# pyannote/pyannote-audio

Hardware: AMD Instinct MI355X
Metric: audio-hours/sec (real-time factor) for speaker-diarization-3.1 pipeline (higher is better)
Workload: dtype f32

## Files before the change

include/pyannote_amd.h:

```cpp
#ifndef PYANNOTE_AMD_H
#define PYANNOTE_AMD_H

#include <stddef.h>
#include <stdint.h>

#ifdef __cplusplus
extern "C" {
#endif

int pa_version(void);
const char* pa_last_error(void);

void pa_prof_enable(int on);
size_t pa_prof_report(char* buf, size_t cap);

#define PA_MAX_LSTM_LAYERS 8
#define PA_MAX_LINEAR 4

typedef struct pa_seg_weights {
  int32_t sinc_stride;
  int32_t lstm_layers;
  int32_t lstm_hidden;
  int32_t lstm_bidir;
  int32_t num_linear;
// ... 101 lines not shown
                   int num_chunks, int num_samples, const float* masks, int num_masks, int mask_frames,
                   const int32_t* nearest_idx, float* emb, void* workspace, size_t workspace_bytes,
                   void* stream);

size_t pa_emb_ragged_workspace_bytes(const pa_emb_weights* w, int num_utterances, int max_samples);
int pa_emb_forward_ragged(const pa_emb_weights* w, const float* wav, int64_t wav_len, const int64_t* offsets,
                          const int32_t* lengths, int num_utterances, int max_samples, const float* masks, float* emb,
                          void* workspace, size_t workspace_bytes, void* stream);

size_t pa_emb_calibrate_workspace_bytes(const pa_emb_weights* w, int num_chunks, int num_samples);
int pa_emb_calibrate_winograd(const pa_emb_weights* w, const float* wav, int64_t wav_len, int64_t chunk_stride,
                              int num_chunks, int num_samples, float* report, float* emb, void* workspace,
                              size_t workspace_bytes, void* stream);
int pa_absmax_diff(const float* got, const float* ref, long n, float* out2, void* stream);

int pa_fbank(const float* wav, long wav_len, long chunk_stride, int B, int N, const float* window,
             const float* tw256, const float* tw512, const float* mel_w, const int* mel_lo,
             const int* mel_hi, int nmel, float* out, int center, void* stream);
int pa_fbank_center_span(const float* fb, int B, int T, int nmel, int kernel, float* out, void* stream);
int pa_resnet_stem(const float* fbank, int B, int T, int F, const float* w9, const float* shift,
                   float* out, void* stream);
int pa_conv3x3(const float* X, int B, int H, int W, int cin, const float* Wg, const float* shift,
               const float* R, float* Y, int cout, int stride, int relu, void* stream);
int pa_winograd_pack_host(const float* conv_weight ,
                          const float* bn_scale , int cout, int cin,
                          float* U_slabs );
int pa_conv3x3_wino(const float* X, int B, int H, int W, int cin, const float* U, const float* shift,
                    const float* R, float* Y, int cout, int relu, void* stream);
int pa_winograd4_pack_host(const float* conv_weight ,
                           const float* bn_scale , int cout, int cin,
                           float* U_slabs );
int pa_conv3x3_wino4(const float* X, int B, int H, int W, int cin, const float* U, const float* shift,
                     const float* R, float* Y, int cout, int relu, void* stream);
int pa_conv3x3_wino4_rows(const float* X, int B, int H, int W, int cin, const float* U, const float* shift,
                          const float* R, float* Y, int cout, int relu, int rows, void* stream);
int pa_conv3x3_wino_rows(const float* X, int B, int H, int W, int cin, const float* U, const float* shift,
                         const float* R, float* Y, int cout, int relu, int y_first, void* stream);
int pa_stats_pool(const float* feat, int B, int Fh, int Tp, int C, const float* masks, int S, int Fm,
                  const int* nearest_idx, float* stats, void* stream);
int pa_fbank_ragged(const float* wav, long wav_len, const int64_t* offsets, const int32_t* lengths, int B,
                    int max_samples, const float* window, const float* tw256, const float* tw512, const float* mel_w,
                    const int* mel_lo, const int* mel_hi, int nmel, float* out, void* stream);
int pa_zero_tail_cols(float* x, int B, int H, int W, int C, const int32_t* lengths, int halvings, void* stream);
int pa_stats_pool_ragged(const float* feat, int B, int Fh, int W, int C, const int32_t* lengths, int halvings,
                         const float* masks, int ld_masks, float* stats, void* stream);

// ... 281 lines not shown
```

pyannote-audio_amd/csrc/emb_conv_s2.hip:

```cpp
#include "common.h"
#include "emb_conv_s2_geom.h"

namespace pa {

typedef __attribute__((address_space(3))) unsigned char* cs2_lds_t;
typedef const volatile f32x4 __attribute__((address_space(3))) * cs2_lds_f32x4_ptr;
__device__ __forceinline__ f32x4 cs2_lds_read128(cs2_lds_t p) { return *(cs2_lds_f32x4_ptr)p; }

__device__ __forceinline__ void cs2_barrier() {
  asm volatile("s_waitcnt lgkmcnt(0)" ::: "memory");
  __builtin_amdgcn_s_barrier();
  asm volatile("" ::: "memory");
}

#define CS2_STR2(x) #x
#define CS2_STR(x) CS2_STR2(x)
#define CS2_TAIL_WAIT_LIT 32
static_assert(ConvS2Geom<4, 1>::TILE_STORES == CS2_TAIL_WAIT_LIT && ConvS2Geom<2, 2>::TILE_STORES == CS2_TAIL_WAIT_LIT,
              "the literal of the s_waitcnt string");
static_assert(ConvS2Geom<4, 1>::NPW <= CS2_SLOTS && ConvS2Geom<2, 2>::NPW <= CS2_SLOTS, "a slot of the MFMA run per piece");

template <int IMM>
__device__ __forceinline__ void cs2_piece(unsigned dst, int voff, __amdgpu_buffer_rsrc_t srd, int soff) {
  asm volatile("s_add_u32 m0, %0, %1\n\ts_nop 0\n\tbuffer_load_dwordx4 %2, %3, %4 offen lds"
               :: "s"(dst), "i"(IMM), "v"(voff), "s"(srd), "s"(soff)
               : "memory", "scc");
}
__device__ __forceinline__ void cs2_piece_s(unsigned dst, int delta, int voff, __amdgpu_buffer_rsrc_t srd, int soff) {
  asm volatile("s_add_u32 m0, %0, %1\n\ts_nop 0\n\tbuffer_load_dwordx4 %2, %3, %4 offen lds"
               :: "s"(dst), "s"(delta), "v"(voff), "s"(srd), "s"(soff)
               : "memory", "scc");
}
struct Cs2Stage {
  __amdgpu_buffer_rsrc_t xsrd, wsrd;
  int soff;
  unsigned pdst, wdst;
  int last_delta;
};
template <class G, int N>
__device__ __forceinline__ void cs2_issue(const Cs2Stage& st, const int (&poff)[G::PPW], const int (&woff)[G::WPW]) {
  if constexpr (N < G::PPW - 1) cs2_piece<4096 * N>(st.pdst, poff[N], st.xsrd, st.soff);
  else if constexpr (N == G::PPW - 1) cs2_piece_s(st.pdst, st.last_delta, poff[N], st.xsrd, st.soff);
  else if constexpr (N < G::NPW) cs2_piece<4096 * (N - G::PPW)>(st.wdst, woff[N - G::PPW], st.wsrd, st.soff);
}
template <class G>
__device__ __forceinline__ void cs2_issue_n(const int n, const Cs2Stage& st, const int (&poff)[G::PPW],
                                            const int (&woff)[G::WPW]) {
  switch (n) {
#define CS2_CASE(I) case I: cs2_issue<G, I>(st, poff, woff); break;
    CS2_CASE(0) CS2_CASE(1) CS2_CASE(2) CS2_CASE(3) CS2_CASE(4) CS2_CASE(5) CS2_CASE(6) CS2_CASE(7) CS2_CASE(8)
    CS2_CASE(9) CS2_CASE(10) CS2_CASE(11) CS2_CASE(12) CS2_CASE(13) CS2_CASE(14) CS2_CASE(15) CS2_CASE(16)
    CS2_CASE(17) CS2_CASE(18) CS2_CASE(19) CS2_CASE(20) CS2_CASE(21) CS2_CASE(22) CS2_CASE(23) CS2_CASE(24)
    CS2_CASE(25) CS2_CASE(26)
#undef CS2_CASE
    default: break;
  }
}

template <int TH, int TWT, bool HAS_R>
__global__ __launch_bounds__(256, 2) void k_conv3x3_s2(const float* __restrict__ X, int H, int W, int CIN,
                                                       const float* __restrict__ Wg,
                                                       const float* __restrict__ shift,
                                                       const float* __restrict__ R, float* __restrict__ Y, int Ho,
                                                       int Wo, int COUT, int relu, int tiles_w, int tiles_hw,
                                                       int n_tiles, int total_tiles, int xranges,
                                                       int* __restrict__ counters) {
  using G = ConvS2Geom<TH, TWT>;
  constexpr int BN = CS2_BN;
  constexpr int OOB = CS2_OOB;
  extern __shared__ __attribute__((aligned(16))) unsigned char smem_s2[];
  const cs2_lds_t lds = (cs2_lds_t)smem_s2;
  const unsigned lds0 = (unsigned)(size_t)lds;
  int* mail = reinterpret_cast<int*>(smem_s2 + G::LDS_BYTES);

  const int tid = threadIdx.x, lane = tid & 63;
  const int slw = __builtin_amdgcn_readfirstlane(tid >> 6);
  const int li = lane & 31, kh = lane >> 5;

  struct Tile {
    int b, n0, y0, x0;
  };
  const int num_pb = total_tiles / n_tiles;
  auto pair_of = [&](int t) {
    return xranges ? (t & 7) * ((num_pb + 7) >> 3) + (t >> 3) / n_tiles : ((t >> 3) / n_tiles) * 8 + (t & 7);
  };
  auto decode = [&](int t) {
    Tile q;
    const int pb = pair_of(t);
    q.n0 = (((t >> 3) % n_tiles)) * BN;
    const int pix = pb % tiles_hw;
// ... 9 lines not shown
      r = tq_claim_own(tqq);
    }
  };

  cs2_lds_t aptr[9][2];
#pragma unroll
  for (int tap = 0; tap < 9; ++tap)
#pragma unroll
    for (int h = 0; h < 2; ++h) {
      aptr[tap][h] = lds + conv_s2_a_addr<G>(slw, li, kh, h, tap);
      asm volatile("" : "+v"(aptr[tap][h]));
    }
  cs2_lds_t bptr[2];
#pragma unroll
  for (int h = 0; h < 2; ++h) {
    bptr[h] = lds + G::W_BASE + conv_s2_b_addr(0, li, kh, h, 0);
    asm volatile("" : "+v"(bptr[h]));
  }
  ConvS2Lane pl[G::PPW];
#pragma unroll
  for (int k = 0; k < G::PPW; ++k) pl[k] = conv_s2_patch_lane<G>(conv_s2_patch_piece<G>(slw, k), lane, W, CIN);
  int woff[G::WPW];
#pragma unroll
  for (int k = 0; k < G::WPW; ++k) woff[k] = conv_s2_w_lane(4 * k + slw, lane, COUT, CIN);
  const int last_delta = 1024 * (conv_s2_patch_piece<G>(slw, G::PPW - 1) - slw);
  int poff[G::PPW];
  auto tile_offsets = [&](const Tile& q) {
    const int sy = 2 * q.y0 - 1, sx = 2 * q.x0 - 1, sbase = conv_s2_tile_base(q.y0, q.x0, W, CIN);
#pragma unroll
    for (int k = 0; k < G::PPW; ++k) poff[k] = conv_s2_patch_off(pl[k], sy, sx, sbase, H, W);
  };
  auto x_srd = [&](const Tile& q, bool live) {
    return __builtin_amdgcn_make_buffer_rsrc(const_cast<float*>(X + (long)q.b * H * W * CIN), 0,
                                             live ? H * W * CIN * 4 : 0, 0x00020000);
  };
  auto w_srd = [&](const Tile& q, bool live) {
    return __builtin_amdgcn_make_buffer_rsrc(const_cast<float*>(Wg + (long)q.n0 * CIN), 0,
                                             live ? (9 * COUT - q.n0) * CIN * 4 : 0, 0x00020000);
  };
  auto stage_to = [&](int to_buf, __amdgpu_buffer_rsrc_t xs, __amdgpu_buffer_rsrc_t ws, int c0) {
    Cs2Stage st;
    st.xsrd = xs;
    st.wsrd = ws;
    st.soff = c0 * 4;
    st.pdst = lds0 + to_buf * G::PATCH_BYTES + 1024 * slw;
    st.wdst = lds0 + G::W_BASE + to_buf * G::W_BYTES + 1024 * slw;
    st.last_delta = __builtin_amdgcn_readfirstlane(last_delta);
    return st;
  };

  const TileQueue tq{counters, (int)(blockIdx.x & 7), ((num_pb + 7) >> 3) * n_tiles};
  if (tid == 0) mail[0] = resolve(tq, tq_claim_own(tq));
  __syncthreads();
  const int t0 = __builtin_amdgcn_readfirstlane(mail[0]);
  if (t0 < 0) {
    if (tid == 0) tq_done(tq, gridDim.x);
    return;
  }
  Tile cur = decode(t0), nxt = cur;
  __amdgpu_buffer_rsrc_t xcur = x_srd(cur, true), wcur = w_srd(cur, true);
  tile_offsets(cur);
  {
    const Cs2Stage st = stage_to(0, xcur, wcur, 0);
#pragma unroll
    for (int n = 0; n < G::NPW; ++n) cs2_issue_n<G>(n, st, poff, woff);
  }
  int claim = 0;
  if (tid == 0) claim = tq_claim_own(tq);
  const int nst = CIN / CS2_CB;
  int buf = 0, tpar = 1, tn = -1;
  bool first_tile = true;

  for (;;) {
    f32x16 acc[2];
#pragma unroll
    for (int j = 0; j < 2; ++j)
#pragma unroll
      for (int r = 0; r < 16; ++r) acc[j][r] = 0.f;
    for (int s = 0; s < nst; ++s) {
      const bool last = s == nst - 1;
      if (s == 0 && !first_tile) asm volatile("s_waitcnt vmcnt(" CS2_STR(CS2_TAIL_WAIT_LIT) ")" ::: "memory");
      else asm volatile("s_waitcnt vmcnt(0)" ::: "memory");
      if (last && tid == 0) mail[tpar] = resolve(tq, claim);
      cs2_barrier();
      Cs2Stage st;
      auto setup = [&]() {
        __amdgpu_buffer_rsrc_t xs = xcur, ws = wcur;
        if (last) {
          tn = __builtin_amdgcn_readfirstlane(mail[tpar]);
          if (tn >= 0) {
            nxt = decode(tn);
            tile_offsets(nxt);
          }
          xs = x_srd(nxt, tn >= 0);
          ws = w_srd(nxt, tn >= 0);
        }
        st = stage_to(buf ^ 1, xs, ws, last ? 0 : (s + 1) * CS2_CB);
      };

      {
        f32x4 fa[2][2], fb[2][2][2];
        auto rd = [&](const int tap, const int r, const int par) {
          const int h = r / 3, w = r % 3;
          if (w == 0) fa[par][h] = cs2_lds_read128(aptr[tap][h]);
          else fb[par][w - 1][h] = cs2_lds_read128(bptr[h] + tap * 4096 + (w - 1) * 2048);
        };
#pragma unroll
        for (int r = 0; r < 6; ++r) rd(0, r, 0);
        __builtin_amdgcn_sched_barrier(0);
        setup();
        __builtin_amdgcn_sched_barrier(0);
#pragma unroll
        for (int tap = 0; tap < 9; ++tap) {
          const int par = tap & 1;
#pragma unroll
          for (int m = 0; m < 16; ++m) {
            const int h = m >> 3, c = (m >> 1) & 3, j = m & 1;
            const float av = fa[par][h][c], bv = fb[par][j][h][c];
            acc[j] = MFMA32(av, bv, acc[j]);
            __builtin_amdgcn_sched_barrier(0);
            if (tap + 1 < 9 && (m & 1) == 0 && m < 12) {
              rd(tap + 1, m >> 1, par ^ 1);
              __builtin_amdgcn_sched_barrier(0);
            }
            const int slot = conv_s2_slot_of(tap, m);
            if (slot >= 0 && slot < G::NPW) {
              cs2_issue_n<G>(slot, st, poff, woff);
              __builtin_amdgcn_sched_barrier(0);
            }
          }
        }
      }
      {
        const int dp = buf ? -G::PATCH_BYTES : G::PATCH_BYTES, dw = buf ? -G::W_BYTES : G::W_BYTES;
#pragma unroll
        for (int tap = 0; tap < 9; ++tap)
#pragma unroll
          for (int h = 0; h < 2; ++h) {
            aptr[tap][h] += dp;
            asm volatile("" : "+v"(aptr[tap][h]));
          }
#pragma unroll
        for (int h = 0; h < 2; ++h) {
          bptr[h] += dw;
// ... 11 lines not shown
          const_cast<float*>(HAS_R ? R + (long)cur.b * Ho * Wo * COUT : Y), 0, Ho * Wo * COUT * 4, 0x00020000);
      const int y = cur.y0 + slw / TWT, xbase = cur.x0 + 32 * (slw % TWT) + 4 * kh;
      int off[2][16];
      float rv[2][16];
      auto goffs = [&](int j, int* o) {
        const int n = cur.n0 + 32 * j + li;
#pragma unroll
        for (int r = 0; r < 16; ++r) {
          const int x = xbase + (r & 3) + 8 * (r >> 2);
          o[r] = (y < Ho && x < Wo) ? ((y * Wo + x) * COUT + n) * 4 : OOB;
        }
      };
      auto gres = [&](const int* o, float* v) {
        if (HAS_R) {
#pragma unroll
          for (int r = 0; r < 16; ++r)
            v[r] = __builtin_bit_cast(float, __builtin_amdgcn_raw_buffer_load_b32(rsrd, o[r], 0, 0));
        } else {
#pragma unroll
          for (int r = 0; r < 16; ++r) v[r] = 0.f;
        }
      };
      const float shv[2] = {shift[cur.n0 + li], shift[cur.n0 + 32 + li]};
      goffs(0, off[0]);
      gres(off[0], rv[0]);
#pragma unroll
      for (int j = 0; j < 2; ++j) {
        if (j + 1 < 2) {
          goffs(j + 1, off[(j + 1) & 1]);
          gres(off[(j + 1) & 1], rv[(j + 1) & 1]);
        }
        const float sh = shv[j];
#pragma unroll
        for (int r = 0; r < 16; ++r) {
          float v = acc[j][r] + sh + rv[j & 1][r];
          if (relu) v = fmaxf(v, 0.f);
          __builtin_amdgcn_raw_buffer_store_b32(__builtin_bit_cast(unsigned int, v), ysrd, off[j & 1][r], 0, 0);
        }
      }
    }
    if (tn < 0) break;
    cur = nxt;
    xcur = x_srd(cur, true);
    wcur = w_srd(cur, true);
    tpar ^= 1;
  }
  if (tid == 0) tq_done(tq, gridDim.x);
}

int xcd_ranges_wanted(bool by_default);

template <int TH, int TWT, bool HAS_R>
static int launch_conv_s2_r(const float* X, int B, int H, int W, int CIN, const float* Wg, const float* shift,
                            const float* R, float* Y, int COUT, int relu, hipStream_t st) {
  using G = ConvS2Geom<TH, TWT>;
  const int Ho = (H - 1) / 2 + 1, Wo = (W - 1) / 2 + 1;
  const int tiles_w = cdiv(Wo, G::TW), tiles_h = cdiv(Ho, TH);
  const size_t lds = (size_t)G::LDS_BYTES + 16;
  constexpr int MAXDEV = 16;
  static int resident_of[MAXDEV] = {0};
  int dev = 0;
  (void)hipGetDevice(&dev);
  if (dev < 0 || dev >= MAXDEV) dev = 0;
  if (!resident_of[dev]) {
    (void)hipFuncSetAttribute((const void*)k_conv3x3_s2<TH, TWT, HAS_R>, hipFuncAttributeMaxDynamicSharedMemorySize,
                              (int)lds);
    int cus = 256;
    (void)hipDeviceGetAttribute(&cus, hipDeviceAttributeMultiprocessorCount, dev);
    resident_of[dev] = cus;
  }
  const int resident = resident_of[dev] & ~7;
  const int tiles_hw = tiles_w * tiles_h, n_tiles = COUT / CS2_BN;
  const long total = (long)tiles_hw * n_tiles * B;
  const int grid = (int)(total < resident ? total : resident);
  int* counters = tile_counters();
  if (counters == nullptr) {
    set_error("pa_conv3x3: cannot allocate the tile counters");
    return 2;
  }
  hipLaunchKernelGGL((k_conv3x3_s2<TH, TWT, HAS_R>), dim3(grid), dim3(256), lds, st, X, H, W, CIN, Wg, shift, R, Y, Ho,
                     Wo, COUT, relu, tiles_w, tiles_hw, n_tiles, (int)total, xcd_ranges_wanted(true), counters);
  return 0;
}

int launch_conv_s2(const float* X, int B, int H, int W, int CIN, const float* Wg, const float* shift, const float* R,
                   float* Y, int COUT, int relu, hipStream_t st) {
  const int Ho = (H - 1) / 2 + 1;
  if (Ho >= 16)
    return R != nullptr ? launch_conv_s2_r<4, 1, true>(X, B, H, W, CIN, Wg, shift, R, Y, COUT, relu, st)
                        : launch_conv_s2_r<4, 1, false>(X, B, H, W, CIN, Wg, shift, R, Y, COUT, relu, st);
  return R != nullptr ? launch_conv_s2_r<2, 2, true>(X, B, H, W, CIN, Wg, shift, R, Y, COUT, relu, st)
                      : launch_conv_s2_r<2, 2, false>(X, B, H, W, CIN, Wg, shift, R, Y, COUT, relu, st);
}

}
```

pyannote-audio_amd/csrc/emb_conv_s2_geom.h:

```cpp
#pragma once

namespace pa {

constexpr int CS2_CB = 16;
constexpr int CS2_BN = 64;
constexpr int CS2_OOB = (int)0x80000000;

template <int TH_, int TWT_>
struct ConvS2Geom {
  static constexpr int TH = TH_, TWT = TWT_, TW = 32 * TWT_;
  static constexpr int PH = 2 * TH + 1, PW = 2 * TW + 1;
  static constexpr int PWH = TW + 1;
  static constexpr int PENT = PH * 2 * PWH;
  static constexpr int PPIECES = (PENT + 15) / 16;
  static constexpr int WPIECES = 9 * CS2_BN / 16;
  static constexpr int PPW = (PPIECES + 3) / 4;
  static constexpr int WPW = WPIECES / 4;
  static constexpr int NPW = PPW + WPW;
  static constexpr int PATCH_BYTES = PPIECES * 1024;
  static constexpr int W_BYTES = WPIECES * 1024;
  static constexpr int W_BASE = 2 * PATCH_BYTES;
  static constexpr int LDS_BYTES = 2 * (PATCH_BYTES + W_BYTES);
  static constexpr int TILE_STORES = 2 * 16;
  static_assert(TH * TWT == 4, "one M-tile per wave, four waves");
  static_assert(WPIECES % 4 == 0 && PPW * 4 >= PPIECES, "pieces split over four waves");
  static_assert(8 * 4096 + 2048 < 65536, "ds_read immediates of a B fragment: tap and N-tile");
  static_assert(LDS_BYTES + 64 <= 160 * 1024, "two stages in LDS");
};

__device__ __forceinline__ int conv_s2_swz(int e) { return (e >> 2) & 3; }

template <class G>
__device__ __forceinline__ int conv_s2_patch_piece(int w, int k) {
  const int i = 4 * k + w;
  return i < G::PPIECES ? i : G::PPIECES - 1;
}

struct ConvS2Lane {
  int rel, py, px;
};
constexpr int CS2_NO_COLUMN = 0x20000000;
template <class G>
__device__ __forceinline__ ConvS2Lane conv_s2_patch_lane(int piece, int lane, int W, int CIN) {
  const int sl = 64 * piece + lane;
  const int e = sl >> 2, q = (sl & 3) ^ conv_s2_swz(e);
  const int plane = e / G::PWH, col = e % G::PWH;
  const int py = plane >> 1, px = 2 * col + (plane & 1);
  const bool real = e < G::PENT && px < G::PW;
  ConvS2Lane L;
  L.rel = ((py * W + px) * CIN + 4 * q) * 4;
  L.py = py;
  L.px = real ? px : CS2_NO_COLUMN;
  return L;
}
__device__ __forceinline__ int conv_s2_tile_base(int y0, int x0, int W, int CIN) {
  return ((2 * y0 - 1) * W + 2 * x0 - 1) * CIN * 4;
}
__device__ __forceinline__ int conv_s2_patch_off(const ConvS2Lane& L, int sy, int sx, int sbase, int H, int W) {
  const bool ok = (unsigned)(L.py + sy) < (unsigned)H && (unsigned)(L.px + sx) < (unsigned)W;
  return ok ? sbase + L.rel : CS2_OOB;
}
__device__ __forceinline__ int conv_s2_w_lane(int piece, int lane, int COUT, int CIN) {
  const int sl = 64 * piece + lane;
  const int e = sl >> 2, q = (sl & 3) ^ conv_s2_swz(e);
  const int tap = e >> 6, n = e & 63;
  return ((tap * COUT + n) * CIN + 4 * q) * 4;
}

template <class G>
__device__ __forceinline__ int conv_s2_a_entry(int mt, int li, int tap) {
  const int dy = tap / 3, dx = tap % 3;
  const int yy = mt / G::TWT, xt = mt % G::TWT;
  return ((2 * yy + dy) * 2 + (dx & 1)) * G::PWH + 32 * xt + li + (dx >> 1);
}
__device__ __forceinline__ int conv_s2_slot_addr(int e, int q) { return e * 64 + ((q ^ conv_s2_swz(e)) << 4); }
template <class G>
__device__ __forceinline__ int conv_s2_a_addr(int mt, int li, int kh, int h, int tap) {
  return conv_s2_slot_addr(conv_s2_a_entry<G>(mt, li, tap), 2 * kh + h);
}
__device__ __forceinline__ int conv_s2_b_addr(int j, int li, int kh, int h, int tap) {
  return conv_s2_slot_addr(tap * 64 + 32 * j + li, 2 * kh + h);
}

constexpr int CS2_SLOTS = 9 * 3;
__device__ __forceinline__ int conv_s2_slot_of(int tap, int m) {
  return (m == 3 || m == 9 || m == 15) ? tap * 3 + (m - 3) / 6 : -1;
}

}
```

pyannote-audio_amd/csrc/emb_forward.cpp:

```cpp
#include "forward_common.h"

namespace {

struct EmbPlan {
  int B, N, T, F, S;
  int Hs[5], Ws[5];
  size_t fbank, act[4], stats, total, act_elems;
  size_t t2_off, gather_off;
};

inline bool prefer_wino4(int H, int W, int cin) {
  auto up = [](int a, int b) { return (long)((a + b - 1) / b) * b; };
  long p4 = up(H, 4) * up(W, 64);
  const long p4_lin = up(H, 4) * up(W, 4);
  if (p4_lin * 120 <= p4 * 100) p4 = p4_lin * 120 / 100;
  long p2 = up(H, 8) * up(W, 32);
  if (up(H, 4) * up(W, 64) < p2) p2 = up(H, 4) * up(W, 64);
  if (up(H, 2) * up(W, 128) < p2) p2 = up(H, 2) * up(W, 128);
  const long gain = cin >= 256 ? 130 : 122;
  return p4 * 100 <= p2 * gain;
}

bool make_plan(const pa_emb_weights* w, int B, int N, int S, EmbPlan* p, bool calib = false) {
  if (N < 400) return false;
  p->B = B;
  p->N = N;
  p->S = S < 1 ? 1 : S;
  p->T = 1 + (N - 400) / 160;
  p->F = w->num_mel;
  p->Hs[0] = p->F;
  p->Ws[0] = p->T;
  for (int l = 0; l < w->num_layers; ++l) {
// ... 161 lines not shown
          pa::set_error("pa_emb_forward: block %d needs a shortcut conv but none was given", blk);
          return 3;
        }
        PA_RUN(pa_gemm_tn_ex(t2, planes, w->blk_w3[blk], planes, w->blk_shift3[blk], res, nxt, cout, B * Ho * Wo,
                             cout, planes, 2, 0, stream));
        float* t = cur;
        cur = nxt;
        nxt = t;
        cin = cout;
      }
    }
  } else
  for (int l = 0; l < w->num_layers; ++l) {
    const int cout = w->planes[l];
    for (int i = 0; i < w->num_blocks[l]; ++i, ++blk) {
      if (blk >= PA_MAX_RES_BLOCKS) {
        pa::set_error("pa_emb_forward: more than %d residual blocks", PA_MAX_RES_BLOCKS);
        return 3;
      }
      const int stride = (i == 0 && l > 0) ? 2 : 1;
      const int H = stride == 2 ? p.Hs[l] : p.Hs[l + 1], W = stride == 2 ? p.Ws[l] : p.Ws[l + 1];
      const int Ho = p.Hs[l + 1], Wo = p.Ws[l + 1];
      if (w->blk_wsc[blk] != nullptr) {
        PA_RUN(pa_conv3x3(cur, B, H, W, cin, w->blk_w1[blk], w->blk_shift1[blk], nullptr, f1, cout, stride,
                          1, stream));
        PA_RUN(zero_tail(f1, l + 1, cout));
        const size_t q = (size_t)B * Ho * Wo * cin;
        float* R = f2 + pa::Bump::align(q);
        if (stride == 2)
          PA_RUN(pa_gemm_tn_s2(cur, B, H, W, cin, w->blk_wsc[blk], cin, w->blk_shiftsc[blk], R, cout, cout, stream));
        else
          PA_RUN(pa_gemm_tn(cur, cin, w->blk_wsc[blk], cin, w->blk_shiftsc[blk], R, cout, B * Ho * Wo, cout, cin, 0, 0,
                            stream));
        PA_RUN(conv_s1(f1, Ho, Wo, cout, w->blk_v2[blk], w->blk_u2[blk], w->blk_w2[blk], w->blk_shift2[blk], R, cur,
                       cout, 2 * blk + 1));
        PA_RUN(zero_tail(cur, l + 1, cout));
      } else {
        if (stride != 1 || cin != cout) {
          pa::set_error("pa_emb_forward: block %d needs a shortcut conv but none was given", blk);
          return 3;
        }
        PA_RUN(conv_s1(cur, H, W, cin, w->blk_v1[blk], w->blk_u1[blk], w->blk_w1[blk], w->blk_shift1[blk], nullptr, f1,
                       cout, 2 * blk));
        PA_RUN(zero_tail(f1, l + 1, cout));
        PA_RUN(conv_s1(f1, H, W, cout, w->blk_v2[blk], w->blk_u2[blk], w->blk_w2[blk], w->blk_shift2[blk], cur, f2,
                       cout, 2 * blk + 1));
        PA_RUN(zero_tail(f2, l + 1, cout));
        float* t = cur;
        cur = f2;
        f2 = t;
      }
      cin = cout;
// ... 62 lines not shown
```

pyannote-audio_amd/csrc/emb_resnet.hip:

```cpp
#include "common.h"

namespace pa {

constexpr int STEM_TS = 64;
constexpr int STEM_LD = STEM_TS + 3;

__global__ __launch_bounds__(256) void k_stem(const float* __restrict__ fb, int T, int F,
                                              const float* __restrict__ w9,
                                              const float* __restrict__ shift,
                                              float* __restrict__ out) {
  extern __shared__ float xs[];
  const int b = blockIdx.y, t0 = blockIdx.x * STEM_TS;
  const int tid = threadIdx.x;
  for (int i = tid; i < 2 * STEM_LD; i += 256) xs[(i < STEM_LD ? 0 : (F + 1) * STEM_LD - STEM_LD) + i] = 0.f;
  const int n = (STEM_TS + 2) * F;
  for (int i0 = 0; i0 < n; i0 += 8 * 256) {
    float v[8];
#pragma unroll
    for (int k = 0; k < 8; ++k) {
      const int i = i0 + tid + 256 * k;
      const int tt = i / F, ff = i - tt * F, t = t0 + tt - 1;
      v[k] = (i < n && t >= 0 && t < T) ? fb[((long)b * T + t) * F + ff] : 0.f;
    }
#pragma unroll
// ... 284 lines not shown
        if (g + 1 < NG) {
          goffs(g + 1, off[(g + 1) & 1]);
          gres(off[(g + 1) & 1], rv[(g + 1) & 1]);
        }
        const int i = g / NT, j = g % NT;
        const float sh = shift[cur.n0 + 32 * j + li];
#pragma unroll
        for (int r = 0; r < 16; ++r) {
          float v = acc[i][j][r] + sh + rv[g & 1][r];
          if (relu) v = fmaxf(v, 0.f);
          __builtin_amdgcn_raw_buffer_store_b32(__builtin_bit_cast(unsigned int, v), ysrd, off[g & 1][r], 0, 0);
        }
      }
    }
    if (tn < 0) break;
    cur = nxt;
  }
  if (tid == 0) tq_done(tq, gridDim.x);
}

int xcd_ranges_wanted(bool by_default);
int launch_conv_s2(const float* X, int B, int H, int W, int CIN, const float* Wg, const float* shift, const float* R,
                   float* Y, int COUT, int relu, hipStream_t st);

template <int TH, int TWT, int BN, bool HAS_R>
static int launch_conv_r(const float* X, int B, int H, int W, int CIN, const float* Wg,
                         const float* shift, const float* R, float* Y, int COUT, int relu,
                         hipStream_t st) {
  using G = ConvGeom<TH, TWT>;
  const int Ho = H, Wo = W;
  const int tiles_w = cdiv(Wo, G::TW), tiles_h = cdiv(Ho, TH);
  const size_t lds = (size_t)(G::PATCH + 9 * BN * CLD) * sizeof(float);
  constexpr int MAXDEV = 16;
  static int resident_of[MAXDEV] = {0}, per_cu_of[MAXDEV] = {0};
  int dev = 0;
  (void)hipGetDevice(&dev);
  if (dev < 0 || dev >= MAXDEV) dev = 0;
  if (!resident_of[dev]) {
    (void)hipFuncSetAttribute((const void*)k_conv3x3<TH, TWT, BN, HAS_R>,
                              hipFuncAttributeMaxDynamicSharedMemorySize, (int)lds);
    int cus = 256, per_cu = 2;
    (void)hipDeviceGetAttribute(&cus, hipDeviceAttributeMultiprocessorCount, dev);
    if (hipOccupancyMaxActiveBlocksPerMultiprocessor(&per_cu, k_conv3x3<TH, TWT, BN, HAS_R>, 256, lds) !=
            hipSuccess || per_cu < 1)
      per_cu = 2;
    resident_of[dev] = cus * per_cu;
// ... 40 lines not shown
int pa_conv3x3(const float* X, int B, int H, int W, int cin, const float* Wg, const float* shift,
               const float* R, float* Y, int cout, int stride, int relu, void* stream) {
  if (B <= 0) return 0;
  PA_REQUIRE(cin % pa::CB == 0 && cout % 32 == 0, "pa_conv3x3: cin %% 16 and cout %% 32 required");
  hipStream_t st = (hipStream_t)stream;
  const int Ho = (H - 1) / stride + 1, Wo_ = (W - 1) / stride + 1;
  pa::ProfScope prof("k_conv3x3", stream, 2.0 * 9 * cin * cout * (double)B * Ho * Wo_,
                     4.0 * ((double)B * H * W * cin + (double)B * Ho * Wo_ * cout * (R ? 2 : 1) + 9.0 * cin * cout));
  if (stride == 1) {
    if (cout == 32) pa::launch_conv<8, 1, 32>(X, B, H, W, cin, Wg, shift, R, Y, cout, relu, st);
    else if (Ho >= 32) pa::launch_conv<8, 1, 64>(X, B, H, W, cin, Wg, shift, R, Y, cout, relu, st);
    else if (Ho >= 16) pa::launch_conv<4, 2, 64>(X, B, H, W, cin, Wg, shift, R, Y, cout, relu, st);
    else pa::launch_conv<2, 2, 64>(X, B, H, W, cin, Wg, shift, R, Y, cout, relu, st);
  } else if (stride == 2) {
    PA_REQUIRE(cout % 64 == 0, "pa_conv3x3: stride 2 needs cout %% 64 == 0");
    if (pa::launch_conv_s2(X, B, H, W, cin, Wg, shift, R, Y, cout, relu, st) != 0) return 2;
  } else {
    PA_REQUIRE(false, "pa_conv3x3: stride %d not supported", stride);
  }
  PA_CHECK_LAUNCH("pa_conv3x3");
  return 0;
}

}
```

pyannote-audio_amd/ffi.py:

```python
from __future__ import annotations

import ctypes as C
from pathlib import Path

import torch

_LIB = None
PA_MAX_LSTM_LAYERS = 8
PA_MAX_LINEAR = 4

c_fp = C.c_void_p


class SegWeights(C.Structure):
    _fields_ = [
        ("sinc_stride", C.c_int32), ("lstm_layers", C.c_int32), ("lstm_hidden", C.c_int32),
        ("lstm_bidir", C.c_int32), ("num_linear", C.c_int32), ("linear_hidden", C.c_int32),
        ("num_classes", C.c_int32), ("num_speakers", C.c_int32),
        ("wav_gamma", C.c_float), ("wav_beta", C.c_float),
        ("sinc_filt", c_fp), ("norm0", c_fp), ("conv1_w", c_fp), ("conv1_b", c_fp), ("norm1", c_fp),
        ("conv2_w", c_fp), ("conv2_b", c_fp), ("norm2", c_fp),
        ("lstm_wih", c_fp * PA_MAX_LSTM_LAYERS), ("lstm_bias", c_fp * PA_MAX_LSTM_LAYERS),
        ("lstm_whh", c_fp * PA_MAX_LSTM_LAYERS),
        ("lin_w", c_fp * PA_MAX_LINEAR), ("lin_b", c_fp * PA_MAX_LINEAR),
# ... 155 lines not shown
    ("pa_emb_ragged_workspace_bytes", [C.POINTER(EmbWeights), C.c_int, C.c_int], C.c_size_t),
    ("pa_emb_forward_ragged", [C.POINTER(EmbWeights), c_fp, C.c_int64, c_fp, c_fp, C.c_int, C.c_int, c_fp, c_fp,
                               c_fp, C.c_size_t, c_fp], C.c_int),
    ("pa_fbank_ragged", [c_fp, C.c_long, c_fp, c_fp, C.c_int, C.c_int, c_fp, c_fp, c_fp, c_fp, c_fp, c_fp, C.c_int,
                         c_fp, c_fp], C.c_int),
    ("pa_zero_tail_cols", [c_fp, C.c_int, C.c_int, C.c_int, C.c_int, c_fp, C.c_int, c_fp], C.c_int),
    ("pa_stats_pool_ragged", [c_fp, C.c_int, C.c_int, C.c_int, C.c_int, c_fp, C.c_int, c_fp, C.c_int, c_fp, c_fp],
     C.c_int),
    ("pa_emb_calibrate_workspace_bytes", [C.POINTER(EmbWeights), C.c_int, C.c_int], C.c_size_t),
    ("pa_emb_calibrate_winograd", [C.POINTER(EmbWeights), c_fp, C.c_int64, C.c_int64, C.c_int, C.c_int, c_fp, c_fp,
                                   c_fp, C.c_size_t, c_fp], C.c_int),
    ("pa_lstm_rec_h", [c_fp, c_fp, c_fp, C.c_int, C.c_int, C.c_int, C.c_int, c_fp], C.c_int),
    ("pa_absmax_diff", [c_fp, c_fp, C.c_long, c_fp, c_fp], C.c_int),
    ("pa_gemm_tn_s2", [c_fp, C.c_int, C.c_int, C.c_int, C.c_int, c_fp, C.c_int, c_fp, c_fp, C.c_long, C.c_int,
                       c_fp], C.c_int),
    ("pa_gemm_tn_batched", [c_fp, C.c_int, C.c_long, C.c_long, c_fp, C.c_int, C.c_long, C.c_long, c_fp, c_fp, C.c_long,
                            C.c_long, C.c_long, C.c_int, C.c_int, C.c_int, C.c_int, C.c_int, C.c_int, c_fp], C.c_int),
    ("pa_fbank", [c_fp, C.c_long, C.c_long, C.c_int, C.c_int, c_fp, c_fp, c_fp, c_fp, c_fp, c_fp,
                  C.c_int, c_fp, C.c_int, c_fp], C.c_int),
    ("pa_fbank_center_span", [c_fp, C.c_int, C.c_int, C.c_int, C.c_int, c_fp, c_fp], C.c_int),
    ("pa_resnet_stem", [c_fp, C.c_int, C.c_int, C.c_int, c_fp, c_fp, c_fp, c_fp], C.c_int),
    ("pa_conv3x3", [c_fp, C.c_int, C.c_int, C.c_int, C.c_int, c_fp, c_fp, c_fp, c_fp, C.c_int, C.c_int,
                    C.c_int, c_fp], C.c_int),
    ("pa_conv3x3_wino", [c_fp, C.c_int, C.c_int, C.c_int, C.c_int, c_fp, c_fp, c_fp, c_fp, C.c_int, C.c_int,
                         c_fp], C.c_int),
    ("pa_conv3x3_wino4", [c_fp, C.c_int, C.c_int, C.c_int, C.c_int, c_fp, c_fp, c_fp, c_fp, C.c_int, C.c_int,
                          c_fp], C.c_int),
    ("pa_conv3x3_wino4_rows", [c_fp, C.c_int, C.c_int, C.c_int, C.c_int, c_fp, c_fp, c_fp, c_fp, C.c_int, C.c_int,
                               C.c_int, c_fp], C.c_int),
    ("pa_conv3x3_wino_rows", [c_fp, C.c_int, C.c_int, C.c_int, C.c_int, c_fp, c_fp, c_fp, c_fp, C.c_int, C.c_int,
                              C.c_int, c_fp], C.c_int),
    ("pa_pdist_f64", [c_fp, C.c_int, C.c_int, c_fp, c_fp], C.c_int),
    ("pa_cdist_cosine_f64", [c_fp, C.c_int, c_fp, C.c_int, C.c_int, c_fp, c_fp, c_fp], C.c_int),
    ("pa_centroid_means", [c_fp, C.c_int, c_fp, c_fp, C.c_int, c_fp, c_fp], C.c_int),
    ("pa_linkage_workspace_bytes", [C.c_int], C.c_size_t),
    ("pa_linkage_centroid_f64", [c_fp, C.c_int, c_fp, c_fp, C.c_size_t, c_fp], C.c_int),
    ("pa_linkage_centroid_f64_ex", [c_fp, C.c_int, c_fp, c_fp, C.c_size_t, C.c_int, c_fp], C.c_int),
    ("pa_pdist_cosine_f64", [c_fp, C.c_int, C.c_int, c_fp, c_fp, c_fp], C.c_int),
    ("pa_nonfinite_flag_f64", [c_fp, C.c_long, c_fp, c_fp], C.c_int),
    ("pa_linkage_chain_workspace_bytes", [C.c_int], C.c_size_t),
    ("pa_linkage_chain_f64", [c_fp, C.c_int, C.c_int, c_fp, c_fp, C.c_size_t, c_fp], C.c_int),
    ("pa_seg_chunk_stats", [c_fp, C.c_int, C.c_int, C.c_int, c_fp, c_fp, c_fp], C.c_int),
    ("pa_embedding_masks", [c_fp, C.c_int, C.c_int, C.c_int, c_fp, C.c_int, C.c_int, c_fp, c_fp], C.c_int),
    ("pa_speaker_count", [c_fp, C.c_int, C.c_int, C.c_int, c_fp, C.c_int, c_fp, c_fp, c_fp], C.c_int),
    ("pa_cluster_activations", [c_fp, C.c_int, C.c_int, C.c_int, c_fp, c_fp, C.c_int, C.c_int, c_fp, c_fp],
     C.c_int),
# ... 144 lines not shown
```

Measured before the change: 1.225.

## Fold 1x1 stride-2 shortcut conv into the stride-2 3x3 conv kernel

Adds a tenth weight tap to the stride-2 3x3 conv kernel that computes the 1x1 stride-2 shortcut projection from the centre tap of the already-staged input patch. The result goes to a second output with its own shift. This removes the separate pa_gemm_tn_s2 launch and its second read of the input activation in downsampling ResNet blocks. In exchange it costs extra LDS for weights, extra accumulators (register pressure at launch_bounds 256,2) and a longer store tail. It is on by default and can be disabled with PA_S2_FOLD=0.

```diff
diff --git a/include/pyannote_amd.h b/include/pyannote_amd.h
--- a/include/pyannote_amd.h
+++ b/include/pyannote_amd.h
@@ -147,6 +147,10 @@
                    float* out, void* stream);
 int pa_conv3x3(const float* X, int B, int H, int W, int cin, const float* Wg, const float* shift,
                const float* R, float* Y, int cout, int stride, int relu, void* stream);
+int pa_conv3x3_s2_sc_supported(int H, int cin, int cout);
+int pa_conv3x3_s2_sc(const float* X, int B, int H, int W, int cin, const float* Wg, const float* shift,
+                     const float* Wsc, const float* shift_sc, float* Y, float* Ysc, int cout, int relu,
+                     void* stream);
 int pa_winograd_pack_host(const float* conv_weight ,
                           const float* bn_scale , int cout, int cin,
                           float* U_slabs );
diff --git a/pyannote-audio_amd/csrc/emb_conv_s2.hip b/pyannote-audio_amd/csrc/emb_conv_s2.hip
--- a/pyannote-audio_amd/csrc/emb_conv_s2.hip
+++ b/pyannote-audio_amd/csrc/emb_conv_s2.hip
@@ -18,7 +18,13 @@
 #define CS2_TAIL_WAIT_LIT 32
 static_assert(ConvS2Geom<4, 1>::TILE_STORES == CS2_TAIL_WAIT_LIT && ConvS2Geom<2, 2>::TILE_STORES == CS2_TAIL_WAIT_LIT,
               "the literal of the s_waitcnt string");
-static_assert(ConvS2Geom<4, 1>::NPW <= CS2_SLOTS && ConvS2Geom<2, 2>::NPW <= CS2_SLOTS, "a slot of the MFMA run per piece");
+#define CS2_TAIL_WAIT_LIT_SC 63
+static_assert(CS2_TAIL_WAIT_LIT_SC <= 63 && ConvS2Geom<4, 1, 1>::TILE_STORES >= CS2_TAIL_WAIT_LIT_SC &&
+                  ConvS2Geom<4, 1, 1>::TILE_STORES == 2 * CS2_TAIL_WAIT_LIT,
+              "the literal of the s_waitcnt string, shortcut folded in: both outputs' stores");
+static_assert(ConvS2Geom<4, 1>::NPW <= CS2_SLOTS && ConvS2Geom<2, 2>::NPW <= CS2_SLOTS &&
+                  ConvS2Geom<4, 1, 1>::NPW <= CS2_SLOTS,
+              "a slot of the MFMA run per piece");
 
 template <int IMM>
 __device__ __forceinline__ void cs2_piece(unsigned dst, int voff, __amdgpu_buffer_rsrc_t srd, int soff) {
@@ -32,7 +38,7 @@
                : "memory", "scc");
 }
 struct Cs2Stage {
-  __amdgpu_buffer_rsrc_t xsrd, wsrd;
+  __amdgpu_buffer_rsrc_t xsrd, wsrd, scsrd;
   int soff;
   unsigned pdst, wdst;
   int last_delta;
@@ -41,6 +47,7 @@
 __device__ __forceinline__ void cs2_issue(const Cs2Stage& st, const int (&poff)[G::PPW], const int (&woff)[G::WPW]) {
   if constexpr (N < G::PPW - 1) cs2_piece<4096 * N>(st.pdst, poff[N], st.xsrd, st.soff);
   else if constexpr (N == G::PPW - 1) cs2_piece_s(st.pdst, st.last_delta, poff[N], st.xsrd, st.soff);
+  else if constexpr (G::SC && N == G::NPW - 1) cs2_piece<4096 * (N - G::PPW)>(st.wdst, woff[N - G::PPW], st.scsrd, st.soff);
   else if constexpr (N < G::NPW) cs2_piece<4096 * (N - G::PPW)>(st.wdst, woff[N - G::PPW], st.wsrd, st.soff);
 }
 template <class G>
@@ -57,15 +64,19 @@
   }
 }
 
-template <int TH, int TWT, bool HAS_R>
+template <int TH, int TWT, bool HAS_R, int SC>
 __global__ __launch_bounds__(256, 2) void k_conv3x3_s2(const float* __restrict__ X, int H, int W, int CIN,
                                                        const float* __restrict__ Wg,
                                                        const float* __restrict__ shift,
                                                        const float* __restrict__ R, float* __restrict__ Y, int Ho,
                                                        int Wo, int COUT, int relu, int tiles_w, int tiles_hw,
                                                        int n_tiles, int total_tiles, int xranges,
-                                                       int* __restrict__ counters) {
-  using G = ConvS2Geom<TH, TWT>;
+                                                       int* __restrict__ counters, const float* __restrict__ Wsc,
+                                                       const float* __restrict__ shift_sc,
+                                                       float* __restrict__ Ysc) {
+  using G = ConvS2Geom<TH, TWT, SC>;
+  static_assert(!(SC && HAS_R), "a block entry has no residual input");
+  constexpr int NT = G::WTAPS;
   constexpr int BN = CS2_BN;
   constexpr int OOB = CS2_OOB;
   extern __shared__ __attribute__((aligned(16))) unsigned char smem_s2[];
@@ -121,7 +132,8 @@
   for (int k = 0; k < G::PPW; ++k) pl[k] = conv_s2_patch_lane<G>(conv_s2_patch_piece<G>(slw, k), lane, W, CIN);
   int woff[G::WPW];
 #pragma unroll
-  for (int k = 0; k < G::WPW; ++k) woff[k] = conv_s2_w_lane(4 * k + slw, lane, COUT, CIN);
+  for (int k = 0; k < G::WPW; ++k)
+    woff[k] = k < 9 ? conv_s2_w_lane(4 * k + slw, lane, COUT, CIN) : conv_s2_wsc_lane(4 * k + slw, lane, CIN);
   const int last_delta = 1024 * (conv_s2_patch_piece<G>(slw, G::PPW - 1) - slw);
   int poff[G::PPW];
   auto tile_offsets = [&](const Tile& q) {
@@ -137,10 +149,16 @@
     return __builtin_amdgcn_make_buffer_rsrc(const_cast<float*>(Wg + (long)q.n0 * CIN), 0,
                                              live ? (9 * COUT - q.n0) * CIN * 4 : 0, 0x00020000);
   };
-  auto stage_to = [&](int to_buf, __amdgpu_buffer_rsrc_t xs, __amdgpu_buffer_rsrc_t ws, int c0) {
+  auto sc_srd = [&](const Tile& q, bool live) {
+    return __builtin_amdgcn_make_buffer_rsrc(const_cast<float*>(SC ? Wsc + (long)q.n0 * CIN : Wg), 0,
+                                             SC && live ? (COUT - q.n0) * CIN * 4 : 0, 0x00020000);
+  };
+  auto stage_to = [&](int to_buf, __amdgpu_buffer_rsrc_t xs, __amdgpu_buffer_rsrc_t ws, __amdgpu_buffer_rsrc_t scs,
+                      int c0) {
     Cs2Stage st;
     st.xsrd = xs;
     st.wsrd = ws;
+    st.scsrd = scs;
     st.soff = c0 * 4;
     st.pdst = lds0 + to_buf * G::PATCH_BYTES + 1024 * slw;
     st.wdst = lds0 + G::W_BASE + to_buf * G::W_BYTES + 1024 * slw;
@@ -157,10 +175,10 @@
     return;
   }
   Tile cur = decode(t0), nxt = cur;
-  __amdgpu_buffer_rsrc_t xcur = x_srd(cur, true), wcur = w_srd(cur, true);
+  __amdgpu_buffer_rsrc_t xcur = x_srd(cur, true), wcur = w_srd(cur, true), sccur = sc_srd(cur, true);
   tile_offsets(cur);
   {
-    const Cs2Stage st = stage_to(0, xcur, wcur, 0);
+    const Cs2Stage st = stage_to(0, xcur, wcur, sccur, 0);
 #pragma unroll
     for (int n = 0; n < G::NPW; ++n) cs2_issue_n<G>(n, st, poff, woff);
   }
@@ -171,20 +189,28 @@
   bool first_tile = true;
 
   for (;;) {
-    f32x16 acc[2];
+    f32x16 acc[2], acc_sc[SC ? 2 : 1];
 #pragma unroll
     for (int j = 0; j < 2; ++j)
 #pragma unroll
       for (int r = 0; r < 16; ++r) acc[j][r] = 0.f;
+#pragma unroll
+    for (int j = 0; j < (SC ? 2 : 0); ++j)
+#pragma unroll
+      for (int r = 0; r < 16; ++r) acc_sc[j][r] = 0.f;
     for (int s = 0; s < nst; ++s) {
       const bool last = s == nst - 1;
-      if (s == 0 && !first_tile) asm volatile("s_waitcnt vmcnt(" CS2_STR(CS2_TAIL_WAIT_LIT) ")" ::: "memory");
-      else asm volatile("s_waitcnt vmcnt(0)" ::: "memory");
+      if (s == 0 && !first_tile) {
+        if constexpr (SC) asm volatile("s_waitcnt vmcnt(" CS2_STR(CS2_TAIL_WAIT_LIT_SC) ")" ::: "memory");
+        else asm volatile("s_waitcnt vmcnt(" CS2_STR(CS2_TAIL_WAIT_LIT) ")" ::: "memory");
+      } else {
+        asm volatile("s_waitcnt vmcnt(0)" ::: "memory");
+      }
       if (last && tid == 0) mail[tpar] = resolve(tq, claim);
       cs2_barrier();
       Cs2Stage st;
       auto setup = [&]() {
-        __amdgpu_buffer_rsrc_t xs = xcur, ws = wcur;
+        __amdgpu_buffer_rsrc_t xs = xcur, ws = wcur, scs = sccur;
         if (last) {
           tn = __builtin_amdgcn_readfirstlane(mail[tpar]);
           if (tn >= 0) {
@@ -193,15 +219,16 @@
           }
           xs = x_srd(nxt, tn >= 0);
           ws = w_srd(nxt, tn >= 0);
-        }
-        st = stage_to(buf ^ 1, xs, ws, last ? 0 : (s + 1) * CS2_CB);
+          scs = sc_srd(nxt, tn >= 0);
+        }
+        st = stage_to(buf ^ 1, xs, ws, scs, last ? 0 : (s + 1) * CS2_CB);
       };
 
       {
         f32x4 fa[2][2], fb[2][2][2];
         auto rd = [&](const int tap, const int r, const int par) {
           const int h = r / 3, w = r % 3;
-          if (w == 0) fa[par][h] = cs2_lds_read128(aptr[tap][h]);
+          if (w == 0) fa[par][h] = cs2_lds_read128(aptr[tap < 9 ? tap : 4][h]);
           else fb[par][w - 1][h] = cs2_lds_read128(bptr[h] + tap * 4096 + (w - 1) * 2048);
         };
 #pragma unroll
@@ -210,15 +237,16 @@
         setup();
         __builtin_amdgcn_sched_barrier(0);
 #pragma unroll
-        for (int tap = 0; tap < 9; ++tap) {
+        for (int tap = 0; tap < NT; ++tap) {
           const int par = tap & 1;
 #pragma unroll
           for (int m = 0; m < 16; ++m) {
             const int h = m >> 3, c = (m >> 1) & 3, j = m & 1;
             const float av = fa[par][h][c], bv = fb[par][j][h][c];
-            acc[j] = MFMA32(av, bv, acc[j]);
+            if (tap < 9) acc[j] = MFMA32(av, bv, acc[j]);
+            else acc_sc[SC ? j : 0] = MFMA32(av, bv, acc_sc[SC ? j : 0]);
             __builtin_amdgcn_sched_barrier(0);
-            if (tap + 1 < 9 && (m & 1) == 0 && m < 12) {
+            if (tap + 1 < NT && (m & 1) == 0 && m < 12) {
               rd(tap + 1, m >> 1, par ^ 1);
               __builtin_amdgcn_sched_barrier(0);
             }
@@ -276,6 +304,13 @@
         }
       };
       const float shv[2] = {shift[cur.n0 + li], shift[cur.n0 + 32 + li]};
+      const __amdgpu_buffer_rsrc_t yscsrd = __builtin_amdgcn_make_buffer_rsrc(
+          SC ? Ysc + (long)cur.b * Ho * Wo * COUT : Y, 0, SC ? Ho * Wo * COUT * 4 : 0, 0x00020000);
+      float shsc[2] = {0.f, 0.f};
+      if constexpr (SC) {
+        shsc[0] = shift_sc[cur.n0 + li];
+        shsc[1] = shift_sc[cur.n0 + 32 + li];
+      }
       goffs(0, off[0]);
       gres(off[0], rv[0]);
 #pragma unroll
@@ -290,6 +325,13 @@
           float v = acc[j][r] + sh + rv[j & 1][r];
           if (relu) v = fmaxf(v, 0.f);
           __builtin_amdgcn_raw_buffer_store_b32(__builtin_bit_cast(unsigned int, v), ysrd, off[j & 1][r], 0, 0);
+        }
+        if constexpr (SC) {
+          const float ss = shsc[j];
+#pragma unroll
+          for (int r = 0; r < 16; ++r)
+            __builtin_amdgcn_raw_buffer_store_b32(__builtin_bit_cast(unsigned int, acc_sc[j][r] + ss), yscsrd,
+                                                  off[j & 1][r], 0, 0);
         }
       }
     }
@@ -297,6 +339,7 @@
     cur = nxt;
     xcur = x_srd(cur, true);
     wcur = w_srd(cur, true);
+    sccur = sc_srd(cur, true);
     tpar ^= 1;
   }
   if (tid == 0) tq_done(tq, gridDim.x);
@@ -304,10 +347,11 @@
 
 int xcd_ranges_wanted(bool by_default);
 
-template <int TH, int TWT, bool HAS_R>
+template <int TH, int TWT, bool HAS_R, int SC = 0>
 static int launch_conv_s2_r(const float* X, int B, int H, int W, int CIN, const float* Wg, const float* shift,
-                            const float* R, float* Y, int COUT, int relu, hipStream_t st) {
-  using G = ConvS2Geom<TH, TWT>;
+                            const float* R, float* Y, int COUT, int relu, hipStream_t st, const float* Wsc = nullptr,
+                            const float* shift_sc = nullptr, float* Ysc = nullptr) {
+  using G = ConvS2Geom<TH, TWT, SC>;
   const int Ho = (H - 1) / 2 + 1, Wo = (W - 1) / 2 + 1;
   const int tiles_w = cdiv(Wo, G::TW), tiles_h = cdiv(Ho, TH);
   const size_t lds = (size_t)G::LDS_BYTES + 16;
@@ -317,7 +361,7 @@
   (void)hipGetDevice(&dev);
   if (dev < 0 || dev >= MAXDEV) dev = 0;
   if (!resident_of[dev]) {
-    (void)hipFuncSetAttribute((const void*)k_conv3x3_s2<TH, TWT, HAS_R>, hipFuncAttributeMaxDynamicSharedMemorySize,
+    (void)hipFuncSetAttribute((const void*)k_conv3x3_s2<TH, TWT, HAS_R, SC>, hipFuncAttributeMaxDynamicSharedMemorySize,
                               (int)lds);
     int cus = 256;
     (void)hipDeviceGetAttribute(&cus, hipDeviceAttributeMultiprocessorCount, dev);
@@ -332,8 +376,9 @@
     set_error("pa_conv3x3: cannot allocate the tile counters");
     return 2;
   }
-  hipLaunchKernelGGL((k_conv3x3_s2<TH, TWT, HAS_R>), dim3(grid), dim3(256), lds, st, X, H, W, CIN, Wg, shift, R, Y, Ho,
-                     Wo, COUT, relu, tiles_w, tiles_hw, n_tiles, (int)total, xcd_ranges_wanted(true), counters);
+  hipLaunchKernelGGL((k_conv3x3_s2<TH, TWT, HAS_R, SC>), dim3(grid), dim3(256), lds, st, X, H, W, CIN, Wg, shift, R, Y,
+                     Ho, Wo, COUT, relu, tiles_w, tiles_hw, n_tiles, (int)total, xcd_ranges_wanted(true), counters, Wsc,
+                     shift_sc, Ysc);
   return 0;
 }
 
@@ -347,4 +392,10 @@
                       : launch_conv_s2_r<2, 2, false>(X, B, H, W, CIN, Wg, shift, R, Y, COUT, relu, st);
 }
 
-}
+int launch_conv_s2_sc(const float* X, int B, int H, int W, int CIN, const float* Wg, const float* shift,
+                      const float* Wsc, const float* shift_sc, float* Y, float* Ysc, int COUT, int relu,
+                      hipStream_t st) {
+  return launch_conv_s2_r<4, 1, false, 1>(X, B, H, W, CIN, Wg, shift, nullptr, Y, COUT, relu, st, Wsc, shift_sc, Ysc);
+}
+
+}
diff --git a/pyannote-audio_amd/csrc/emb_conv_s2_geom.h b/pyannote-audio_amd/csrc/emb_conv_s2_geom.h
--- a/pyannote-audio_amd/csrc/emb_conv_s2_geom.h
+++ b/pyannote-audio_amd/csrc/emb_conv_s2_geom.h
@@ -6,14 +6,15 @@
 constexpr int CS2_BN = 64;
 constexpr int CS2_OOB = (int)0x80000000;
 
-template <int TH_, int TWT_>
+template <int TH_, int TWT_, int SC_ = 0>
 struct ConvS2Geom {
-  static constexpr int TH = TH_, TWT = TWT_, TW = 32 * TWT_;
+  static constexpr int TH = TH_, TWT = TWT_, TW = 32 * TWT_, SC = SC_;
+  static constexpr int WTAPS = 9 + SC_;
   static constexpr int PH = 2 * TH + 1, PW = 2 * TW + 1;
   static constexpr int PWH = TW + 1;
   static constexpr int PENT = PH * 2 * PWH;
   static constexpr int PPIECES = (PENT + 15) / 16;
-  static constexpr int WPIECES = 9 * CS2_BN / 16;
+  static constexpr int WPIECES = WTAPS * CS2_BN / 16;
   static constexpr int PPW = (PPIECES + 3) / 4;
   static constexpr int WPW = WPIECES / 4;
   static constexpr int NPW = PPW + WPW;
@@ -21,10 +22,11 @@
   static constexpr int W_BYTES = WPIECES * 1024;
   static constexpr int W_BASE = 2 * PATCH_BYTES;
   static constexpr int LDS_BYTES = 2 * (PATCH_BYTES + W_BYTES);
-  static constexpr int TILE_STORES = 2 * 16;
+  static constexpr int TILE_STORES = 2 * 16 * (1 + SC_);
+  static_assert(SC_ == 0 || SC_ == 1, "the shortcut is there or not");
   static_assert(TH * TWT == 4, "one M-tile per wave, four waves");
   static_assert(WPIECES % 4 == 0 && PPW * 4 >= PPIECES, "pieces split over four waves");
-  static_assert(8 * 4096 + 2048 < 65536, "ds_read immediates of a B fragment: tap and N-tile");
+  static_assert((WTAPS - 1) * 4096 + 2048 < 65536, "ds_read immediates of a B fragment: tap and N-tile");
   static_assert(LDS_BYTES + 64 <= 160 * 1024, "two stages in LDS");
 };
 
@@ -66,6 +68,12 @@
   const int tap = e >> 6, n = e & 63;
   return ((tap * COUT + n) * CIN + 4 * q) * 4;
 }
+__device__ __forceinline__ int conv_s2_wsc_lane(int piece, int lane, int CIN) {
+  const int sl = 64 * piece + lane;
+  const int e = sl >> 2, q = (sl & 3) ^ conv_s2_swz(e);
+  const int n = e & 63;
+  return (n * CIN + 4 * q) * 4;
+}
 
 template <class G>
 __device__ __forceinline__ int conv_s2_a_entry(int mt, int li, int tap) {
diff --git a/pyannote-audio_amd/csrc/emb_forward.cpp b/pyannote-audio_amd/csrc/emb_forward.cpp
--- a/pyannote-audio_amd/csrc/emb_forward.cpp
+++ b/pyannote-audio_amd/csrc/emb_forward.cpp
@@ -8,6 +8,11 @@
   size_t fbank, act[4], stats, total, act_elems;
   size_t t2_off, gather_off;
 };
+
+inline bool s2_fold_wanted() {
+  static const bool fold = getenv("PA_S2_FOLD") == nullptr || atoi(getenv("PA_S2_FOLD")) != 0;
+  return fold;
+}
 
 inline bool prefer_wino4(int H, int W, int cin) {
   auto up = [](int a, int b) { return (long)((a + b - 1) / b) * b; };
@@ -215,12 +220,18 @@
       const int H = stride == 2 ? p.Hs[l] : p.Hs[l + 1], W = stride == 2 ? p.Ws[l] : p.Ws[l + 1];
       const int Ho = p.Hs[l + 1], Wo = p.Ws[l + 1];
       if (w->blk_wsc[blk] != nullptr) {
-        PA_RUN(pa_conv3x3(cur, B, H, W, cin, w->blk_w1[blk], w->blk_shift1[blk], nullptr, f1, cout, stride,
-                          1, stream));
-        PA_RUN(zero_tail(f1, l + 1, cout));
         const size_t q = (size_t)B * Ho * Wo * cin;
         float* R = f2 + pa::Bump::align(q);
-        if (stride == 2)
+        const bool fold = stride == 2 && s2_fold_wanted() && pa_conv3x3_s2_sc_supported(H, cin, cout);
+        if (fold)
+          PA_RUN(pa_conv3x3_s2_sc(cur, B, H, W, cin, w->blk_w1[blk], w->blk_shift1[blk], w->blk_wsc[blk],
+                                  w->blk_shiftsc[blk], f1, R, cout, 1, stream));
+        else
+          PA_RUN(pa_conv3x3(cur, B, H, W, cin, w->blk_w1[blk], w->blk_shift1[blk], nullptr, f1, cout, stride,
+                            1, stream));
+        PA_RUN(zero_tail(f1, l + 1, cout));
+        if (fold) {
+        } else if (stride == 2)
           PA_RUN(pa_gemm_tn_s2(cur, B, H, W, cin, w->blk_wsc[blk], cin, w->blk_shiftsc[blk], R, cout, cout, stream));
         else
           PA_RUN(pa_gemm_tn(cur, cin, w->blk_wsc[blk], cin, w->blk_shiftsc[blk], R, cout, B * Ho * Wo, cout, cin, 0, 0,
diff --git a/pyannote-audio_amd/csrc/emb_resnet.hip b/pyannote-audio_amd/csrc/emb_resnet.hip
--- a/pyannote-audio_amd/csrc/emb_resnet.hip
+++ b/pyannote-audio_amd/csrc/emb_resnet.hip
@@ -330,6 +330,9 @@
 int xcd_ranges_wanted(bool by_default);
 int launch_conv_s2(const float* X, int B, int H, int W, int CIN, const float* Wg, const float* shift, const float* R,
                    float* Y, int COUT, int relu, hipStream_t st);
+int launch_conv_s2_sc(const float* X, int B, int H, int W, int CIN, const float* Wg, const float* shift,
+                      const float* Wsc, const float* shift_sc, float* Y, float* Ysc, int COUT, int relu,
+                      hipStream_t st);
 
 template <int TH, int TWT, int BN, bool HAS_R>
 static int launch_conv_r(const float* X, int B, int H, int W, int CIN, const float* Wg,
@@ -416,4 +419,27 @@
   return 0;
 }
 
-}
+int pa_conv3x3_s2_sc_supported(int H, int cin, int cout) {
+  return H >= 1 && cin >= pa::CB && cin % pa::CB == 0 && cout >= 64 && cout % 64 == 0 && (H - 1) / 2 + 1 >= 16;
+}
+
+int pa_conv3x3_s2_sc(const float* X, int B, int H, int W, int cin, const float* Wg, const float* shift,
+                     const float* Wsc, const float* shift_sc, float* Y, float* Ysc, int cout, int relu,
+                     void* stream) {
+  if (B <= 0) return 0;
+  PA_REQUIRE(cin >= pa::CB && cin % pa::CB == 0, "pa_conv3x3_s2_sc: cin %% 16 == 0 required");
+  PA_REQUIRE(cout >= 64 && cout % 64 == 0, "pa_conv3x3_s2_sc: cout %% 64 == 0 required");
+  const int Ho = (H - 1) / 2 + 1, Wo_ = (W - 1) / 2 + 1;
+  PA_REQUIRE(H >= 1 && W >= 1 && Ho >= 16, "pa_conv3x3_s2_sc: at least 16 output rows required (got %d)", Ho);
+  const size_t n_out = (size_t)B * Ho * Wo_ * cout;
+  PA_REQUIRE(Y != nullptr && Ysc != nullptr && (Y + n_out <= Ysc || Ysc + n_out <= Y),
+             "pa_conv3x3_s2_sc: Y and Ysc overlap");
+  pa::ProfScope prof("k_conv3x3", stream, 2.0 * (9 + 1) * cin * cout * (double)B * Ho * Wo_,
+                     4.0 * ((double)B * H * W * cin + 2.0 * (double)B * Ho * Wo_ * cout + 10.0 * cin * cout));
+  if (pa::launch_conv_s2_sc(X, B, H, W, cin, Wg, shift, Wsc, shift_sc, Y, Ysc, cout, relu, (hipStream_t)stream) != 0)
+    return 2;
+  PA_CHECK_LAUNCH("pa_conv3x3_s2_sc");
+  return 0;
+}
+
+}
diff --git a/pyannote-audio_amd/ffi.py b/pyannote-audio_amd/ffi.py
--- a/pyannote-audio_amd/ffi.py
+++ b/pyannote-audio_amd/ffi.py
@@ -201,6 +201,9 @@
     ("pa_resnet_stem", [c_fp, C.c_int, C.c_int, C.c_int, c_fp, c_fp, c_fp, c_fp], C.c_int),
     ("pa_conv3x3", [c_fp, C.c_int, C.c_int, C.c_int, C.c_int, c_fp, c_fp, c_fp, c_fp, C.c_int, C.c_int,
                     C.c_int, c_fp], C.c_int),
+    ("pa_conv3x3_s2_sc_supported", [C.c_int, C.c_int, C.c_int], C.c_int),
+    ("pa_conv3x3_s2_sc", [c_fp, C.c_int, C.c_int, C.c_int, C.c_int, c_fp, c_fp, c_fp, c_fp, c_fp, c_fp, C.c_int,
+                          C.c_int, c_fp], C.c_int),
     ("pa_conv3x3_wino", [c_fp, C.c_int, C.c_int, C.c_int, C.c_int, c_fp, c_fp, c_fp, c_fp, C.c_int, C.c_int,
                          c_fp], C.c_int),
     ("pa_conv3x3_wino4", [c_fp, C.c_int, C.c_int, C.c_int, C.c_int, c_fp, c_fp, c_fp, c_fp, C.c_int, C.c_int,
```

Result: faster. 1.237, median of 6 (+1.0%).
